# CompVis/stable-diffusion

Measured on AMD Instinct MI355X. Metric: 512x512 images/sec, SD-v1-4 50-step PLMS CFG=7.5, higher is better.
Workload: dtype f16

## Files before the change

stable-diffusion_amd/csrc/conv3halo.hip:

```cpp
#include "igemm_dev.h"

namespace sdmi {
namespace {

template <int BM, int BN, int WARPS_M, int WARPS_N, int NS>
__global__ void __launch_bounds__(WARPS_M* WARPS_N * 64) conv3halo_kernel(const IGemmParams p, const int tiles_m,
                                                                           const int tiles_n, const int chunks_per_split) {
#if defined(__HIP_DEVICE_COMPILE__)
  constexpr int NT = WARPS_M * WARPS_N * 64;
  constexpr int RPP = NT / 8;
  constexpr int PB = BN / RPP;
  constexpr int WTM = BM / WARPS_M, WTN = BN / WARPS_N;
  constexpr int TM = WTM / 32, TN = WTN / 32;
  constexpr int HPMAX = (BM / 64 + 2) * 66;
  constexpr int AHP = (HPMAX + RPP - 1) / RPP;
  constexpr int HALO_BYTES = AHP * RPP * 128;
  constexpr int BSTAGE = BN * 128;
  constexpr int LDS_BYTES = 2 * HALO_BYTES + NS * BSTAGE;
  constexpr int LASTA = 10 - NS;
  constexpr int PA = (AHP + LASTA) / (LASTA + 1);
  constexpr int KS = BK / 16;
  constexpr int G = (TM * TN >= 4) ? 1 : 2;
  constexpr int U = KS / G;
  constexpr int MPU = G * TM * TN;
  static_assert(PB >= 1 && TM >= 1 && TN >= 1 && RPP % 16 == 0 && NS >= 2 && NS <= 9, "tile/wave shape");
  static_assert(LDS_BYTES <= 160 * 1024, "LDS budget");

  __shared__ __attribute__((aligned(16))) unsigned char smem[LDS_BYTES];

  const int nblk = gridDim.x;
  const int bid = blockIdx.x;
  const int q8 = nblk >> 3, r8 = nblk & 7, xcd = bid & 7;
  const int wgid = (xcd < r8 ? xcd * (q8 + 1) : r8 * (q8 + 1) + (xcd - r8) * q8) + (bid >> 3);
  const int tiles_mn = tiles_m * tiles_n;
  const int split = wgid / tiles_mn;
  const int tmn = wgid - split * tiles_mn;
  int tile_m, tile_n;
  if (p.tile_n_fastest) { tile_m = tmn / tiles_n; tile_n = tmn - tile_m * tiles_n; }
  else { tile_n = tmn / tiles_m; tile_m = tmn - tile_n * tiles_m; }
  const int m0 = tile_m * BM, n0 = tile_n * BN;
  const int nch = (p.c0 + p.c1 + p.c2) / BK;
  const int c_begin = split * chunks_per_split;
  const int c_end = min(nch, c_begin + chunks_per_split);
  if (c_begin >= c_end) return;

  const int tid = threadIdx.x;
  SDMI_STAMP(dbg_t0);
  const int lane = tid & 63;
  const int wave = tid >> 6;
  const int cpos = tid & 7, lrow = tid >> 3;
  const int gch = cpos ^ ((lrow >> 1) & 7);
  const int wave_u = __builtin_amdgcn_readfirstlane(wave);
  const int wm = wave / WARPS_N, wn = wave - wm * WARPS_N;
  const int l31 = lane & 31, lg = lane >> 5;
  const int rsw = (l31 >> 1) & 7;

  const int W = p.Wout, H = p.Hout, HW = H * W, W2 = W + 2, ld = p.lda0;
  const int bimg = m0 / HW;
// ... 60 lines not shown
      for (int r = 0; r < 16; ++r) acc[i][j][r] = 0.f;

  auto a_base = [&](int i, int ky, int kx, int hbuf) -> int {
    const int rowt = hr0[i] + ky * W2 + kx;
    return hbuf * HALO_BYTES + ((rowt << 7) | ((lg ^ ((rowt >> 1) & 7)) << 4));
  };
  auto read_frags = [&](const int (&ab)[TM], int bstage, int ks, f16x8 (&a)[TM], f16x8 (&b)[TN]) {
#pragma unroll
    for (int i = 0; i < TM; ++i) a[i] = *(const f16x8*)(smem + (ab[i] ^ (ks << 5)));
    const unsigned char* st = smem + bstage * BSTAGE + b_lds + (((ks * 2 + lg) ^ rsw) << 4);
#pragma unroll
    for (int j = 0; j < TN; ++j) b[j] = *(const f16x8*)(st + j * 32 * 128);
  };
  auto mfma_step = [&](const f16x8 (&a)[TM], const f16x8 (&b)[TN]) {
#pragma unroll
    for (int i = 0; i < TM; ++i)
#pragma unroll
      for (int j = 0; j < TN; ++j) acc[i][j] = __builtin_amdgcn_mfma_f32_32x32x16_f16(a[i], b[j], acc[i][j], 0, 0, 0);
  };

  auto a_lo = [](int t) { return t <= LASTA ? (t * PA < AHP ? t * PA : AHP) : AHP; };
  auto a_hi = [](int t) { return t <= LASTA ? ((t + 1) * PA < AHP ? (t + 1) * PA : AHP) : AHP; };
  auto in_flight_ok = [&](int t) {
    int n = 0;
    for (int d = 0; d < NS - 2; ++d) { const int tt = (t - d + 18) % 9; n += a_hi(tt) - a_lo(tt) + PB; }
    return n;
  };

  const int kt_first = c_begin * 9, kt_last = c_end * 9 - 1;
  {
    const ChunkSrc cs = chunk_src(c_begin);
#pragma unroll
    for (int q = 0; q < AHP; ++q) issue_halo(cs, 0, q);
#pragma unroll
    for (int s2 = 0; s2 < NS - 1; ++s2) {
      const int vt = 9 - (NS - 1) + s2;
#pragma unroll
      for (int e = a_lo(vt); e < a_hi(vt); ++e) issue_halo(cs, 0, 0);
#pragma unroll
      for (int q = 0; q < PB; ++q) issue_b(min(kt_first + s2, kt_last), s2, q);
    }
  }
  wait_vmcnt_n(in_flight_ok(8));
  asm volatile("s_waitcnt lgkmcnt(0)\n\ts_barrier" ::: "memory");
  SDMI_STAMP(dbg_t1);
  f16x8 fa[2][G][TM], fb[2][G][TN];
  int ab[TM];
#pragma unroll
  for (int i = 0; i < TM; ++i) ab[i] = a_base(i, 0, 0, 0);
#pragma unroll
  for (int g = 0; g < G; ++g) read_frags(ab, 0, g, fa[0][g], fb[0][g]);

  int cur = 0, nxt = NS - 1, hb = 0;
  for (int c = c_begin; c < c_end; ++c) {
    const ChunkSrc csn = chunk_src(min(c + 1, c_end - 1));
#pragma unroll
    for (int tap = 0; tap < 9; ++tap) {
      const int kt = c * 9 + tap;
      const int tap1 = tap == 8 ? 0 : tap + 1;
      const int hb1 = tap == 8 ? (hb ^ 1) : hb;
      const int cur1 = (cur + 1 == NS) ? 0 : cur + 1;
      int ab1[TM];
#pragma unroll
      for (int i = 0; i < TM; ++i) ab1[i] = a_base(i, tap1 / 3, tap1 % 3, hb1);
      const int alo = a_lo(tap);
      const int na = a_hi(tap) - alo;
      const int npieces = na + PB;
      const int ppu = (npieces + U - 2) / (U - 1);
      const int bt = min(kt + NS - 1, kt_last);
#pragma unroll
      for (int u = 0; u < U; ++u) {
        if (u + 1 < U) {
#pragma unroll
          for (int g = 0; g < G; ++g) read_frags(ab, cur, (u + 1) * G + g, fa[(u + 1) & 1][g], fb[(u + 1) & 1][g]);
#pragma unroll
          for (int e = u * ppu; e < (u + 1) * ppu && e < npieces; ++e) {
            if (e < na) issue_halo(csn, hb ^ 1, alo + e);
            else issue_b(bt, nxt, e - na);
          }
        } else {
          wait_vmcnt_n(in_flight_ok(tap));
          asm volatile("s_waitcnt lgkmcnt(0)\n\ts_barrier" ::: "memory");
#pragma unroll
          for (int g = 0; g < G; ++g) read_frags(ab1, cur1, g, fa[0][g], fb[0][g]);
        }
#pragma unroll
        for (int g = 0; g < G; ++g) mfma_step(fa[u & 1][g], fb[u & 1][g]);
        __builtin_amdgcn_sched_group_barrier(0x100, G * (TM + TN), 0);
#pragma unroll
        for (int e = 0; e < MPU; ++e) {
          __builtin_amdgcn_sched_group_barrier(0x008, 1, 0);
          if (u + 1 < U && e < ppu && u * ppu + e < npieces) __builtin_amdgcn_sched_group_barrier(0x010, 1, 0);
        }
      }
#pragma unroll
      for (int i = 0; i < TM; ++i) ab[i] = ab1[i];
      cur = cur1;
      nxt = (nxt + 1 == NS) ? 0 : nxt + 1;
      hb = hb1;
    }
  }
  wait_vmcnt<0>();
  SDMI_STAMP(dbg_t2);
  igemm_epilogue<BM, BN, WARPS_M, WARPS_N, LDS_BYTES>(p, acc, m0, n0, split, tile_m, tile_n, smem);
#ifdef SDMI_IGEMM_TIMING
  if (p.dbg_times && tid == 0) {
    long long* d = p.dbg_times + 6 * (size_t)blockIdx.x;
    d[0] = dbg_t0; d[1] = dbg_t1; d[2] = dbg_t2; d[4] = (long long)__builtin_readcyclecounter();
  }
#endif
#endif
}

}

bool halo_supported(const IGemmParams& p, int bm) {
  const int W = p.Wout, HW = p.Hout * p.Wout;
  if (p.c0 % BK || p.c1 % BK || p.c2 % BK) return false;
  if (!(p.ksize == 3 && p.stride == 1 && p.pad == 1 && !p.up && p.Hin == p.Hout && p.Win == p.Wout && W >= 8 && W <= 64 &&
        (W & (W - 1)) == 0 && bm % W == 0))
    return false;
  const int cap = (((bm / 64 + 2) * 66 + bm / 4 - 1) / (bm / 4)) * (bm / 4);
  if (bm <= HW) return HW % bm == 0 && (bm / W + 2) * (W + 2) <= cap;
  return bm % HW == 0 && p.M % bm == 0 && (bm / HW) * (p.Hout + 2) * (W + 2) <= cap;
}

template <int BM, int BN, int WARPS_M, int WARPS_N, int NS>
int launch_halo_cfg(const IGemmParams& p, int splitk, hipStream_t stream) {
  SDMI_CHECK(halo_supported(p, BM), "halo-staged conv tile requested for an unsupported shape");
  const int tiles_m = cdiv(p.M, BM), tiles_n = cdiv(p.N, BN);
  const int nch = (p.c0 + p.c1 + p.c2) / BK;
  const int chunks_per_split = cdiv(nch, splitk);
  const int nsplit = cdiv(nch, chunks_per_split);
  IGemmParams q = p;
  q.splitk = nsplit;
  q.tile_n_fastest = tile_order_n_fastest(p);
  q.splitk_fused = 0;
  slab_layout(q, BM, BN, WARPS_M, WARPS_N, nsplit);
  q.epi_vec = epi_vec_ok(p);
  SDMI_CHECK(splitk_ws_need(p, BM, BN, nsplit) <= p.splitk_ws_floats, "split-K workspace too small");
  SDMI_CHECK((int64_t)p.M < (int64_t)65536 * p.Hout * p.Wout, "fast_div_hw: at most 65535 samples per launch");
  q.magic_hw = div_magic_hw(p.Hout * p.Wout);
  q.magic_w = div_magic(p.Wout);
  q.magic_w2 = div_magic(p.Wout + 2);
  q.log2w = 0;
  while ((1 << q.log2w) < p.Wout) ++q.log2w;
  {
    const int HW = p.Hout * p.Wout;
    q.halo_ipt = BM <= HW ? 1 : BM / HW;
    q.halo_thi = BM <= HW ? BM / p.Wout : p.Hout;
    q.magic_hpi = div_magic((q.halo_thi + 2) * (p.Wout + 2));
    const int tpi = q.halo_thi * p.Wout;
    q.log2_tpi = 0;
    while ((1 << q.log2_tpi) < tpi) ++q.log2_tpi;
    if (q.halo_ipt == 1) q.log2_tpi = 30;
  }
  for (int t = 0; t < p.gn_n; ++t) q.gn_magic[t] = div_magic(p.gn_cpg[t]);
  dim3 grid(tiles_m * tiles_n * nsplit), block(WARPS_M * WARPS_N * 64);
  static const int by_shape = env_int("SDMI_PROF_SHAPES", 0);
  std::string pname = std::string("conv3halo_") + std::to_string(BM) + "x" + std::to_string(BN) + "w" +
                      std::to_string(WARPS_M * WARPS_N) + "s" + std::to_string(NS);
  if (by_shape && prof_enabled())
    pname += "_M" + std::to_string(p.M) + "_N" + std::to_string(p.N) + "_K" + std::to_string(p.K) + "_s" + std::to_string(nsplit);
  const double src_pix = (double)p.B * p.Hin * p.Win;
  ProfScope ps(pname.c_str(), 2.0 * p.M * (double)p.N * p.K,
               src_pix * (p.c0 + p.c1) * 2.0 + (double)p.N * p.K * 2.0 + (double)p.M * p.N * ((p.out_f32 ? 4.0 : 0.0) + (p.out_f16 ? 2.0 : 0.0)) +
                   (p.residual ? (double)p.M * p.N * 4.0 : 0.0),
               stream);
  SDMI_LAUNCH((conv3halo_kernel<BM, BN, WARPS_M, WARPS_N, NS>), grid, block, 0, stream, q, tiles_m, tiles_n, chunks_per_split);
  SDMI_HIP_OK(hipGetLastError());
  ps.end();
  if (nsplit > 1) return launch_splitk_reduce(q, nsplit, stream);
  if (q.ln_out) return launch_layernorm(q.out_f32, q.ln_gamma, q.ln_beta, q.ln_out, q.M, q.N, q.ln_eps, stream);
  return 0;
}

int launch_halo_tile(int tile, const IGemmParams& p, int splitk, hipStream_t stream) {
  switch (tile) {
    case 14: return launch_halo_cfg<256, 64, 4, 2, 5>(p, splitk, stream);
    case 15: return launch_halo_cfg<256, 128, 4, 2, 3>(p, splitk, stream);
    case 16: return launch_halo_cfg<128, 64, 2, 2, 8>(p, splitk, stream);
    case 17: return launch_halo_cfg<128, 128, 2, 2, 5>(p, splitk, stream);
    default: return fail("not a halo-staged conv tile id");
  }
}

}
```

stable-diffusion_amd/csrc/gemm_split16.hip:

```cpp
#include "igemm_dev.h"

namespace sdmi {
namespace {

template <int BM, int BN, int WARPS_M, int WARPS_N, int NS, bool HALF>
__global__ void __launch_bounds__(WARPS_M* WARPS_N * 64) gemm_split16_kernel(const IGemmParams p, const int tiles_m, const int tiles_n,
                                                                               const int kt_per_split) {
#if defined(__HIP_DEVICE_COMPILE__)
  constexpr int NT = WARPS_M * WARPS_N * 64;
  constexpr int RPP = NT / 8;
  constexpr int A_PASSES = BM / RPP, B_PASSES = BN / RPP;
  constexpr int WTM = BM / WARPS_M, WTN = BN / WARPS_N;
  constexpr int TM = WTM / 32, TN = WTN / 32;
  constexpr int A_BYTES = BM * 128, B_BYTES = BN * 128;
  constexpr int STAGE_BYTES = 2 * (A_BYTES + B_BYTES);
  constexpr int LPT = 2 * (A_PASSES + B_PASSES);
  constexpr int KS = BK / 16;
  constexpr int PPU = (LPT + KS - 2) / (KS - 1);
  static_assert(A_PASSES >= 1 && B_PASSES >= 1 && TM >= 1 && TN >= 1 && RPP % 16 == 0 && NS >= 2, "tile/wave shape");
  static_assert(NS * STAGE_BYTES <= 160 * 1024, "LDS budget");

  __shared__ __attribute__((aligned(16))) unsigned char smem[NS * STAGE_BYTES];

  const int nblk = gridDim.x, bid = blockIdx.x;
  const int q8 = nblk >> 3, r8 = nblk & 7, xcd = bid & 7;
  const int wgid = (xcd < r8 ? xcd * (q8 + 1) : r8 * (q8 + 1) + (xcd - r8) * q8) + (bid >> 3);
  const int tiles_mn = tiles_m * tiles_n;
  const int split = wgid / tiles_mn;
  const int tmn = wgid - split * tiles_mn;
  int tile_m, tile_n;
  if (p.tile_n_fastest) { tile_m = tmn / tiles_n; tile_n = tmn - tile_m * tiles_n; }
  else { tile_n = tmn / tiles_m; tile_m = tmn - tile_n * tiles_m; }
  const int m0 = tile_m * BM, n0 = tile_n * BN;
  const int nkt = HALF ? p.nkt : p.K / BK;
  const int kt_begin = split * kt_per_split;
  const int kt_end = min(nkt, kt_begin + kt_per_split);
  if (kt_begin >= kt_end) return;

  const int tid = threadIdx.x;
  SDMI_STAMP(dbg_t0);
  const int lane = tid & 63, wave = tid >> 6;
  const int cpos = tid & 7, lrow = tid >> 3;
  const int gch = cpos ^ ((lrow >> 1) & 7);
  const int hi_oob = (HALF && gch >= 4) ? (int)0x80000000 : 0;
  const int kt_half = HALF ? nkt - 1 : -1;
  const int wave_u = __builtin_amdgcn_readfirstlane(wave);

  int a_off[A_PASSES], b_off[B_PASSES];
#pragma unroll
  for (int i = 0; i < A_PASSES; ++i) a_off[i] = (min(m0 + i * RPP + lrow, p.M - 1) * p.lda0 + gch * 8) * 2;
#pragma unroll
  for (int i = 0; i < B_PASSES; ++i) b_off[i] = (min(n0 + i * RPP + lrow, p.N - 1) * p.ldw + gch * 8) * 2;
  constexpr int OOB = (int)0x80000000;
  const __amdgpu_buffer_rsrc_t rsrc_hi = __builtin_amdgcn_make_buffer_rsrc((void*)p.a0, 0, OOB, 0x00020000);
  const __amdgpu_buffer_rsrc_t rsrc_lo = __builtin_amdgcn_make_buffer_rsrc((void*)p.a1, 0, OOB, 0x00020000);
  const __amdgpu_buffer_rsrc_t rsrc_w = __builtin_amdgcn_make_buffer_rsrc((void*)p.w, 0, OOB, 0x00020000);
  const int w_lo_off = 2 * p.K * 2;

  auto issue_piece = [&](int kt, int stage, int q) {
    const int soff = kt * (BK * 2);
    const int half = HALF ? (hi_oob & (kt == kt_half ? (int)0x80000000 : 0)) : 0;
    const bool isA = q < 2 * A_PASSES;
    const int qa = isA ? q : q - 2 * A_PASSES;
    const int npass = isA ? A_PASSES : B_PASSES;
    const int hl = qa >= npass ? 1 : 0, pass = qa - hl * npass;
    const unsigned row0 = (isA ? hl * BM : 2 * BM + hl * BN) + pass * RPP + wave_u * 8;
    auto dst = (__attribute__((address_space(3))) void*)(smem + stage * STAGE_BYTES + row0 * 128);
    if (isA) __builtin_amdgcn_raw_ptr_buffer_load_lds(hl ? rsrc_lo : rsrc_hi, dst, 16, a_off[pass] | half, soff, 0, 0);
    else __builtin_amdgcn_raw_ptr_buffer_load_lds(rsrc_w, dst, 16, b_off[pass] | half, soff + (hl ? w_lo_off : 0), 0, SDMI_W_AUX);
  };

  const int wm = wave / WARPS_N, wn = wave - wm * WARPS_N;
  const int l31 = lane & 31, lg = lane >> 5;
  const int rsw = (l31 >> 1) & 7;
  f32x16 acc[TM][TN];
#pragma unroll
  for (int i = 0; i < TM; ++i)
#pragma unroll
    for (int j = 0; j < TN; ++j)
#pragma unroll
      for (int r = 0; r < 16; ++r) acc[i][j][r] = 0.f;

  struct Frags { f16x8 ah[TM], al[TM], bh[TN], bl[TN]; };
  const int a_lds = (wm * WTM + l31) * 128, b_lds = 2 * A_BYTES + (wn * WTN + l31) * 128;
  auto read_frags = [&](int stage, int ks, Frags& f) {
    const unsigned char* st = smem + stage * STAGE_BYTES + (((ks * 2 + lg) ^ rsw) << 4);
#pragma unroll
    for (int i = 0; i < TM; ++i) {
      f.ah[i] = *(const f16x8*)(st + a_lds + i * 32 * 128);
      f.al[i] = *(const f16x8*)(st + a_lds + A_BYTES + i * 32 * 128);
    }
#pragma unroll
    for (int j = 0; j < TN; ++j) {
      f.bh[j] = *(const f16x8*)(st + b_lds + j * 32 * 128);
      f.bl[j] = *(const f16x8*)(st + b_lds + B_BYTES + j * 32 * 128);
    }
  };
  auto mfma_step = [&](const Frags& f) {
#pragma unroll
    for (int i = 0; i < TM; ++i)
#pragma unroll
      for (int j = 0; j < TN; ++j) {
        acc[i][j] = __builtin_amdgcn_mfma_f32_32x32x16_f16(f.ah[i], f.bh[j], acc[i][j], 0, 0, 0);
        acc[i][j] = __builtin_amdgcn_mfma_f32_32x32x16_f16(f.al[i], f.bh[j], acc[i][j], 0, 0, 0);
        acc[i][j] = __builtin_amdgcn_mfma_f32_32x32x16_f16(f.ah[i], f.bl[j], acc[i][j], 0, 0, 0);
      }
  };

  SDMI_STAMP(dbg_t1);
  int ld_kt = kt_begin;
  auto next_kt = [&]() { const int k = ld_kt; if (ld_kt + 1 < kt_end) ++ld_kt; return k; };
#pragma unroll
  for (int s = 0; s < NS - 1; ++s) {
    const int k = next_kt();
#pragma unroll
    for (int q = 0; q < LPT; ++q) issue_piece(k, s, q);
  }
  wait_vmcnt<LPT*(NS - 2)>();
  asm volatile("s_waitcnt lgkmcnt(0)\n\ts_barrier" ::: "memory");
  Frags fr[2];
  read_frags(0, 0, fr[0]);
  int cur = 0, nxt = NS - 1;
  for (int kt = kt_begin; kt < kt_end; ++kt) {
    const int kload = next_kt();
    const int cur1 = (cur + 1 == NS) ? 0 : cur + 1;
#pragma unroll
    for (int u = 0; u < KS; ++u) {
      if (u + 1 < KS) {
        read_frags(cur, u + 1, fr[(u + 1) & 1]);
#pragma unroll
        for (int q = u * PPU; q < (u + 1) * PPU && q < LPT; ++q) issue_piece(kload, nxt, q);
      } else {
        wait_vmcnt<LPT*(NS - 2)>();
        asm volatile("s_waitcnt lgkmcnt(0)\n\ts_barrier" ::: "memory");
        read_frags(cur1, 0, fr[0]);
      }
      mfma_step(fr[u & 1]);
      __builtin_amdgcn_sched_group_barrier(0x100, 2 * (TM + TN), 0);
#pragma unroll
      for (int e = 0; e < 3 * TM * TN; ++e) {
        __builtin_amdgcn_sched_group_barrier(0x008, 1, 0);
        if (u + 1 < KS && e < PPU && u * PPU + e < LPT) __builtin_amdgcn_sched_group_barrier(0x010, 1, 0);
      }
    }
    cur = cur1;
    nxt = (nxt + 1 == NS) ? 0 : nxt + 1;
  }
  wait_vmcnt<0>();
  SDMI_STAMP(dbg_t2);
  igemm_epilogue<BM, BN, WARPS_M, WARPS_N, NS * STAGE_BYTES>(p, acc, m0, n0, split, tile_m, tile_n, smem);
#ifdef SDMI_IGEMM_TIMING
  if (p.dbg_times && tid == 0) {
    long long* d = p.dbg_times + 6 * (size_t)blockIdx.x;
    d[0] = dbg_t0; d[1] = dbg_t1; d[2] = dbg_t2; d[4] = (long long)__builtin_readcyclecounter();
  }
#endif
#endif
}

template <int BM, int BN, int WARPS_M, int WARPS_N, int NS>
int launch_split16_cfg(const IGemmParams& p, int splitk, hipStream_t stream) {
  const int tiles_m = cdiv(p.M, BM), tiles_n = cdiv(p.N, BN);
  const int nkt = igemm_nkt(p);
  const int kt_per_split = cdiv(nkt, splitk);
  const int nsplit = cdiv(nkt, kt_per_split);
  IGemmParams q = p;
  q.nkt = nkt;
  q.splitk = nsplit;
  q.tile_n_fastest = tile_order_n_fastest(p);
  q.splitk_fused = 0;
  slab_layout(q, BM, BN, WARPS_M, WARPS_N, nsplit);
  q.epi_vec = epi_vec_ok(p);
  SDMI_CHECK(splitk_ws_need(p, BM, BN, nsplit) <= p.splitk_ws_floats, "split-K workspace too small");
  SDMI_CHECK((int64_t)p.M < (int64_t)65536 * p.Hout * p.Wout, "fast_div_hw: at most 65535 samples per launch");
  q.magic_hw = div_magic_hw(p.Hout * p.Wout);
  q.magic_w = div_magic(p.Wout);
  for (int t = 0; t < p.gn_n; ++t) q.gn_magic[t] = div_magic(p.gn_cpg[t]);
  dim3 grid(tiles_m * tiles_n * nsplit), block(WARPS_M * WARPS_N * 64);
  static const int by_shape = env_int("SDMI_PROF_SHAPES", 0);
  std::string pname = std::string("gemm_split16_") + std::to_string(BM) + "x" + std::to_string(BN) + "w" +
                      std::to_string(WARPS_M * WARPS_N) + "s" + std::to_string(NS);
  if (by_shape && prof_enabled())
    pname += "_M" + std::to_string(p.M) + "_N" + std::to_string(p.N) + "_K" + std::to_string(p.K) + "_s" + std::to_string(nsplit);
  ProfScope ps(pname.c_str(), 2.0 * p.M * (double)p.N * p.K,
               (double)p.M * p.K * 2.0 + (double)p.N * p.K * 2.0 + (double)p.M * p.N * ((p.out_f32 ? 4.0 : 0.0) + (p.out_f16 ? 2.0 : 0.0)) +
                   (p.residual ? (double)p.M * p.N * 4.0 : 0.0),
               stream, 6.0 * p.M * (double)p.N * p.K);
  if (igemm_has_half(p)) SDMI_LAUNCH((gemm_split16_kernel<BM, BN, WARPS_M, WARPS_N, NS, true>), grid, block, 0, stream, q, tiles_m, tiles_n, kt_per_split);
  else SDMI_LAUNCH((gemm_split16_kernel<BM, BN, WARPS_M, WARPS_N, NS, false>), grid, block, 0, stream, q, tiles_m, tiles_n, kt_per_split);
  SDMI_HIP_OK(hipGetLastError());
  ps.end();
  if (nsplit > 1) return launch_splitk_reduce(q, nsplit, stream);
  if (q.ln_out) return launch_layernorm(q.out_f32, q.ln_gamma, q.ln_beta, q.ln_out, q.M, q.N, q.ln_eps, stream);
  return 0;
}

}

bool split16_tile_supported(int tile) { return tile == 0 || tile == 1 || tile == 2 || tile == 4 || tile == 5 || tile == 8 || tile == 10; }

int launch_split16_tile(int tile, const IGemmParams& p, int splitk, hipStream_t stream) {
  SDMI_CHECK(p.a0 && p.a1 && p.ksize == 1 && p.mode == EPI_PLAIN && p.c1 == 0 && p.c2 == 0 && p.K == p.c0 && p.K % BKH == 0 &&
                 p.lda0 % 8 == 0 && p.ldw % 8 == 0 && p.ldw >= 3 * p.K,
             "split-fp16 GEMM: hi + lo operands, plain epilogue, K % 32 == 0, packed [N][3K] weights");
  switch (tile) {
    case 0: return launch_split16_cfg<128, 128, 2, 2, 2>(p, splitk, stream);
    case 1: return launch_split16_cfg<128, 64, 2, 2, 2>(p, splitk, stream);
    case 2: return launch_split16_cfg<64, 64, 2, 2, 2>(p, splitk, stream);
    case 4: return launch_split16_cfg<128, 64, 2, 2, 3>(p, splitk, stream);
    case 5: return launch_split16_cfg<64, 64, 2, 2, 3>(p, splitk, stream);
    case 8: return launch_split16_cfg<64, 128, 2, 2, 3>(p, splitk, stream);
    case 10: return launch_split16_cfg<64, 64, 2, 2, 4>(p, splitk, stream);
    default: return fail("split-fp16 GEMM: tile id without an instantiation");
  }
}

}
```

stable-diffusion_amd/csrc/igemm_dev.h:

```cpp
#pragma once
#include "common.h"
#include "prof.h"

namespace sdmi {
typedef unsigned u32x4 __attribute__((ext_vector_type(4)));

int launch_splitk_reduce(const IGemmParams& p, int nsplit, hipStream_t stream);
int launch_generic_tile_g0(int tile, const IGemmParams& p, bool dma, int splitk, hipStream_t stream);
int launch_generic_tile_g1(int tile, const IGemmParams& p, bool dma, int splitk, hipStream_t stream);
int launch_generic_tile_g2(int tile, const IGemmParams& p, bool dma, int splitk, hipStream_t stream);
int launch_generic_tile_h0(int tile, const IGemmParams& p, bool dma, int splitk, hipStream_t stream);
int launch_generic_tile_h1(int tile, const IGemmParams& p, bool dma, int splitk, hipStream_t stream);
int launch_generic_tile_h2(int tile, const IGemmParams& p, bool dma, int splitk, hipStream_t stream);

static int env_int(const char* name, int dflt) {
  const char* v = getenv(name);
  return v ? atoi(v) : dflt;
}

namespace {

constexpr int BK = 64;
constexpr int BKH = 32;
static inline int src_chunks(int c) { return (c + BK - 1) / BK; }
static inline bool igemm_has_half(const IGemmParams& p) { return p.split16 ? (p.K % BK != 0) : (p.c0 % BK || p.c1 % BK || p.c2 % BK); }
static inline int igemm_nkt(const IGemmParams& p) {
  if (p.split16) return src_chunks(p.K);
  return p.ksize * p.ksize * (src_chunks(p.c0) + src_chunks(p.c1) + src_chunks(p.c2));
}

#ifdef SDMI_IGEMM_TIMING
#define SDMI_STAMP(name) const long long name = p.dbg_times ? (long long)__builtin_readcyclecounter() : 0
#else
#define SDMI_STAMP(name)
#endif

__device__ __forceinline__ float gelu_erf(float x) {
  const float z = fabsf(x) * 0.70710678118654752440f;
  const float t = __builtin_amdgcn_rcpf(1.0f + 0.3275911f * z);
  const float poly = t * (0.254829592f + t * (-0.284496736f + t * (1.421413741f + t * (-1.453152027f + t * 1.061405429f))));
  const float erf_abs = 1.0f - poly * __expf(-z * z);
  const float erf_v = __builtin_copysignf(erf_abs, x);
  return 0.5f * x * (1.0f + erf_v);
}

__device__ __forceinline__ void wait_vmcnt_n(int n) {
  switch (n) {
#define SDMI_VMCNT_CASE(k) case k: asm volatile("s_waitcnt vmcnt(" #k ")" ::: "memory"); break
    SDMI_VMCNT_CASE(0); SDMI_VMCNT_CASE(1); SDMI_VMCNT_CASE(2); SDMI_VMCNT_CASE(3); SDMI_VMCNT_CASE(4);
    SDMI_VMCNT_CASE(5); SDMI_VMCNT_CASE(6); SDMI_VMCNT_CASE(7); SDMI_VMCNT_CASE(8); SDMI_VMCNT_CASE(9);
    SDMI_VMCNT_CASE(10); SDMI_VMCNT_CASE(11); SDMI_VMCNT_CASE(12); SDMI_VMCNT_CASE(13); SDMI_VMCNT_CASE(14);
    SDMI_VMCNT_CASE(15); SDMI_VMCNT_CASE(16); SDMI_VMCNT_CASE(17); SDMI_VMCNT_CASE(18); SDMI_VMCNT_CASE(19);
    SDMI_VMCNT_CASE(20); SDMI_VMCNT_CASE(21); SDMI_VMCNT_CASE(22); SDMI_VMCNT_CASE(23); SDMI_VMCNT_CASE(24);
    SDMI_VMCNT_CASE(25); SDMI_VMCNT_CASE(26); SDMI_VMCNT_CASE(27); SDMI_VMCNT_CASE(28); SDMI_VMCNT_CASE(29);
    SDMI_VMCNT_CASE(30); SDMI_VMCNT_CASE(31); SDMI_VMCNT_CASE(32); SDMI_VMCNT_CASE(33); SDMI_VMCNT_CASE(34);
    SDMI_VMCNT_CASE(35); SDMI_VMCNT_CASE(36); SDMI_VMCNT_CASE(37); SDMI_VMCNT_CASE(38); SDMI_VMCNT_CASE(39);
    SDMI_VMCNT_CASE(40); SDMI_VMCNT_CASE(41); SDMI_VMCNT_CASE(42); SDMI_VMCNT_CASE(43); SDMI_VMCNT_CASE(44);
    SDMI_VMCNT_CASE(45); SDMI_VMCNT_CASE(46); SDMI_VMCNT_CASE(47); SDMI_VMCNT_CASE(48);
#undef SDMI_VMCNT_CASE
    default: __builtin_trap();
  }
}
template <int N>
__device__ __forceinline__ void wait_vmcnt() {
  static_assert(N >= 0 && N <= 48, "add the literal");
  wait_vmcnt_n(N);
}

enum : int { KIND_1X1 = 0, KIND_3X3 = 1, KIND_3X3_UP = 2 };

__device__ __forceinline__ int fast_div(int m, unsigned long long magic) {
// ... 583 lines not shown
```

stable-diffusion_amd/csrc/igemm_kernel.h:

```cpp
#pragma once
#include <string>

#include "igemm_dev.h"

namespace sdmi {
namespace {


template <int BM, int BN, int WARPS_M, int WARPS_N, bool DMA, int NS, int KIND, bool HALF = false>
__global__ void __launch_bounds__(WARPS_M* WARPS_N * 64) igemm_kernel(const IGemmParams p, const int tiles_m,
                                                                       const int tiles_n, const int kt_per_split) {
  static_assert(DMA || NS == 2, "the register-staged path is double buffered");
#if defined(__HIP_DEVICE_COMPILE__)
  constexpr bool UP = KIND == KIND_3X3_UP;
  constexpr bool K3 = KIND != KIND_1X1;
  constexpr int NT = WARPS_M * WARPS_N * 64;
  constexpr int RPP = NT / 8;
  constexpr int A_PASSES = BM / RPP;
  constexpr int B_PASSES = BN / RPP;
  constexpr int WTM = BM / WARPS_M, WTN = BN / WARPS_N;
  constexpr int TM = WTM / 32, TN = WTN / 32;
  constexpr int STAGE_BYTES = (BM + BN) * 128;
  static_assert(A_PASSES >= 1 && B_PASSES >= 1 && TM >= 1 && TN >= 1, "tile/wave shape");
  static_assert(RPP % 16 == 0, "swizzle assumes pass offset keeps row bits 1..3");

  __shared__ __attribute__((aligned(16))) unsigned char smem[NS * STAGE_BYTES];

  const int nblk = gridDim.x;
  const int bid = blockIdx.x;
  const int q8 = nblk >> 3, r8 = nblk & 7, xcd = bid & 7;
  const int wgid = (xcd < r8 ? xcd * (q8 + 1) : r8 * (q8 + 1) + (xcd - r8) * q8) + (bid >> 3);
  const int tiles_mn = tiles_m * tiles_n;
  const int split = wgid / tiles_mn;
  const int tmn = wgid - split * tiles_mn;
  int tile_m, tile_n;
  if (p.tile_n_fastest) { tile_m = tmn / tiles_n; tile_n = tmn - tile_m * tiles_n; }
  else { tile_n = tmn / tiles_m; tile_m = tmn - tile_n * tiles_m; }
  const int m0 = tile_m * BM, n0 = tile_n * BN;
  const int nkt = HALF ? p.nkt : p.K / BK;
  const int kt_begin = split * kt_per_split;
  const int kt_end = min(nkt, kt_begin + kt_per_split);
  if (kt_begin >= kt_end) return;

  const int tid = threadIdx.x;
  SDMI_STAMP(dbg_t0);
  float2 lnf_pv[LNF_MAXP];
  float lnf_mean = 0.f, lnf_rstd = 1.f;
  const bool lnf_mine = p.lnf_part != nullptr && tid < BM;
  if (lnf_mine) lnf_request(p, min(m0 + tid, p.M - 1), lnf_pv);
  const int lane = tid & 63;
  const int wave = tid >> 6;
  const int cpos = tid & 7;
  const int lrow = tid >> 3;
  const int gch = cpos ^ ((lrow >> 1) & 7);
  const int hi_oob = (HALF && gch >= 4) ? (int)0x80000000 : 0;

  const int HWout = p.Hout * p.Wout;
  const int pad = K3 ? p.pad : 0;
  constexpr int ntap = K3 ? 9 : 1;
  const int ld = p.lda0;
  int a_off[A_PASSES];
  unsigned a_mask[K3 ? A_PASSES : 1];
// ... 51 lines not shown
  int ld_ky = K3 ? ld_tap / 3 : 0, ld_kx = K3 ? ld_tap - 3 * (ld_tap / 3) : 0;
  const int pc0 = p.c0, pc1 = p.c1, pc2 = p.c2;
  const int pp0 = (pc0 + BK - 1) & ~(BK - 1), pp01 = pp0 + ((pc1 + BK - 1) & ~(BK - 1));
  int ld_boff = 0;
  if constexpr (HALF) {
    const int dense0 = ld_cin0 - (ld_cin0 >= pp0 ? pp0 - pc0 : 0) - (ld_cin0 >= pp01 ? pp01 - pp0 - pc1 : 0);
    const int left = ld_cin0 < pp0 ? pc0 - ld_cin0 : (ld_cin0 < pp01 ? pc1 - (ld_cin0 - pp0) : pc2 - (ld_cin0 - pp01));
    ld_boff = (ntap * dense0 + ld_tap * min(left, BK)) * 2;
  }

  constexpr int OOB = (int)0x80000000;
  const long long a_shift = (K3 && !UP) ? (long long)(pad * p.Win + pad) * ld * 2 : 0;
  const char* const srcA0 = (const char*)p.a0 - a_shift; const char* const srcA1 = (const char*)p.a1 - a_shift;
  const char* const srcA2 = (const char*)p.a2 - a_shift;
  const __amdgpu_buffer_rsrc_t rsrc_w = __builtin_amdgcn_make_buffer_rsrc((void*)p.w, 0, OOB, 0x00020000);
  const int pWin = p.Win;

  struct TileCursor { __amdgpu_buffer_rsrc_t rsrc_a; int a_soff, b_soff; unsigned tapbit; int ky, kx; unsigned lds; int half; };
  auto next_tile = [&](int stage) {
    TileCursor c;
    const char* src; int coff, left;
    if (ld_cin0 < pp0) { src = srcA0; coff = ld_cin0; left = pc0 - coff; }
    else if (ld_cin0 < pp01) { src = srcA1; coff = ld_cin0 - pp0; left = pc1 - coff; }
    else { src = srcA2; coff = ld_cin0 - pp01; left = pc2 - coff; }
    const bool half = HALF && left < BK;
    c.rsrc_a = __builtin_amdgcn_make_buffer_rsrc((void*)src, 0, OOB, 0x00020000);
    c.a_soff = ((K3 && !UP) ? (ld_ky * pWin + ld_kx) * ld + coff : coff) * 2;
    c.b_soff = HALF ? ld_boff : ld_kt * (BK * 2);
    c.tapbit = 1u << (half ? ld_tap + 9 : ld_tap); c.ky = ld_ky; c.kx = ld_kx;
    c.half = half ? OOB : 0;
    c.lds = stage * STAGE_BYTES;
    if (ld_kt + 1 < kt_end) {
      ++ld_kt;
      if constexpr (HALF) ld_boff += half ? BKH * 2 : BK * 2;
      if constexpr (K3) {
        ++ld_tap;
        if (++ld_kx == 3) { ld_kx = 0; ++ld_ky; }
        if (ld_tap == ntap) { ld_tap = 0; ld_ky = 0; ld_kx = 0; ld_cin0 += BK; }
      } else {
        ld_cin0 += BK;
      }
    }
    return c;
  };
  auto a_voff = [&](const TileCursor& c, int i) -> int {
    int v;
    if constexpr (UP) v = a_ro[i][c.ky] + a_co[i][c.kx];
    else v = a_off[i];
    if constexpr (K3) v = (a_mask[i] & c.tapbit) ? v : OOB;
    else if constexpr (HALF) v |= hi_oob & c.half;
    return v;
  };
  auto b_voff = [&](const TileCursor& c, int i) -> int { return HALF ? (b_off[i] | (hi_oob & c.half)) : b_off[i]; };
  auto issue_piece = [&](const TileCursor& c, int q) {
    const unsigned row0 = (q < A_PASSES ? q * RPP : BM + (q - A_PASSES) * RPP) + wave_u * 8;
    auto dst = (__attribute__((address_space(3))) void*)(smem + c.lds + row0 * 128);
    if (q < A_PASSES) __builtin_amdgcn_raw_ptr_buffer_load_lds(c.rsrc_a, dst, 16, a_voff(c, q), c.a_soff, 0, 0);
    else __builtin_amdgcn_raw_ptr_buffer_load_lds(rsrc_w, dst, 16, b_voff(c, q - A_PASSES), c.b_soff, 0, SDMI_W_AUX);
  };
  auto issue_loads = [&](int stage) {
    const TileCursor c = next_tile(stage);
#pragma unroll
    for (int q = 0; q < A_PASSES + B_PASSES; ++q) {
      if constexpr (DMA) {
        issue_piece(c, q);
      } else {
        typedef int i32x4 __attribute__((ext_vector_type(4)));
        i32x4 v;
        if (q < A_PASSES) v = __builtin_amdgcn_raw_buffer_load_b128(c.rsrc_a, a_voff(c, q), c.a_soff, 0);
        else v = __builtin_amdgcn_raw_buffer_load_b128(rsrc_w, b_voff(c, q - A_PASSES), c.b_soff, 0);
        if (q < A_PASSES) regA[q] = __builtin_bit_cast(f16x8, v);
        else regB[q - A_PASSES] = __builtin_bit_cast(f16x8, v);
      }
    }
  };
  auto commit_regs = [&](int stage) {
    if constexpr (!DMA) {
      unsigned char* As = smem + stage * STAGE_BYTES;
      unsigned char* Bs = As + BM * 128;
#pragma unroll
      for (int i = 0; i < A_PASSES; ++i) *(f16x8*)(As + (i * RPP + lrow) * 128 + cpos * 16) = regA[i];
#pragma unroll
      for (int i = 0; i < B_PASSES; ++i) *(f16x8*)(Bs + (i * RPP + lrow) * 128 + cpos * 16) = regB[i];
    }
  };

  const int wm = wave / WARPS_N, wn = wave - wm * WARPS_N;
  const int l31 = lane & 31, lg = lane >> 5;
  const int rsw = (l31 >> 1) & 7;
  f32x16 acc[TM][TN];
#pragma unroll
  for (int i = 0; i < TM; ++i)
#pragma unroll
    for (int j = 0; j < TN; ++j)
#pragma unroll
      for (int r = 0; r < 16; ++r) acc[i][j][r] = 0.f;

  const int a_lds = (wm * WTM + l31) * 128, b_lds = BM * 128 + (wn * WTN + l31) * 128;
  auto read_frags = [&](int stage, int ks, f16x8 (&a)[TM], f16x8 (&b)[TN]) {
    const unsigned char* st = smem + stage * STAGE_BYTES + (((ks * 2 + lg) ^ rsw) << 4);
#pragma unroll
    for (int i = 0; i < TM; ++i) a[i] = *(const f16x8*)(st + a_lds + i * 32 * 128);
#pragma unroll
    for (int j = 0; j < TN; ++j) b[j] = *(const f16x8*)(st + b_lds + j * 32 * 128);
  };
  auto mfma_step = [&](const f16x8 (&a)[TM], const f16x8 (&b)[TN]) {
#pragma unroll
    for (int i = 0; i < TM; ++i)
#pragma unroll
      for (int j = 0; j < TN; ++j) acc[i][j] = __builtin_amdgcn_mfma_f32_32x32x16_f16(a[i], b[j], acc[i][j], 0, 0, 0);
  };

  SDMI_STAMP(dbg_t1);
  if constexpr (!DMA) { if (lnf_mine) lnf_finish(p, lnf_pv, &lnf_mean, &lnf_rstd); }
  if constexpr (DMA) {
    constexpr int LPT = A_PASSES + B_PASSES;
    constexpr int KS = BK / 16;
    constexpr int G = (TM * TN >= 4) ? 1 : 2;
    constexpr int U = KS / G;
    constexpr int PPU = (LPT + U - 2) / (U - 1);
    constexpr int MPU = G * TM * TN;
#pragma unroll
    for (int s = 0; s < NS - 1; ++s) issue_loads(s);
    if (p.lnf_part) { wait_vmcnt<0>(); if (lnf_mine) lnf_finish(p, lnf_pv, &lnf_mean, &lnf_rstd); }
    wait_vmcnt<LPT*(NS - 2)>();
    asm volatile("s_waitcnt lgkmcnt(0)\n\ts_barrier" ::: "memory");
    f16x8 fa[2][G][TM], fb[2][G][TN];
#pragma unroll
    for (int g = 0; g < G; ++g) read_frags(0, g, fa[0][g], fb[0][g]);
    int cur = 0, nxt = NS - 1;
    for (int kt = kt_begin; kt < kt_end; ++kt) {
      const TileCursor c = next_tile(nxt);
      const int cur1 = (cur + 1 == NS) ? 0 : cur + 1;
#pragma unroll
      for (int u = 0; u < U; ++u) {
        if (u + 1 < U) {
#pragma unroll
          for (int g = 0; g < G; ++g) read_frags(cur, (u + 1) * G + g, fa[(u + 1) & 1][g], fb[(u + 1) & 1][g]);
#pragma unroll
          for (int q = u * PPU; q < (u + 1) * PPU && q < LPT; ++q) issue_piece(c, q);
        } else {
          wait_vmcnt<LPT*(NS - 2)>();
          asm volatile("s_waitcnt lgkmcnt(0)\n\ts_barrier" ::: "memory");
#pragma unroll
          for (int g = 0; g < G; ++g) read_frags(cur1, g, fa[0][g], fb[0][g]);
        }
#pragma unroll
        for (int g = 0; g < G; ++g) mfma_step(fa[u & 1][g], fb[u & 1][g]);
        __builtin_amdgcn_sched_group_barrier(0x100, G * (TM + TN), 0);
#pragma unroll
        for (int e = 0; e < MPU; ++e) {
          __builtin_amdgcn_sched_group_barrier(0x008, 1, 0);
          if (u + 1 < U && e < PPU && u * PPU + e < LPT) __builtin_amdgcn_sched_group_barrier(0x010, 1, 0);
        }
      }
      cur = cur1;
      nxt = (nxt + 1 == NS) ? 0 : nxt + 1;
    }
    wait_vmcnt<0>();
  } else {
    issue_loads(0);
    commit_regs(0);
    for (int kt = kt_begin; kt < kt_end; ++kt) {
      const int cur = (kt - kt_begin) & 1;
      __syncthreads();
      const bool more = (kt + 1 < kt_end);
      if (more) issue_loads(cur ^ 1);
#pragma unroll
      for (int ks = 0; ks < BK / 16; ++ks) {
        f16x8 a[TM], b[TN];
        read_frags(cur, ks, a, b);
        mfma_step(a, b);
      }
      if (more) commit_regs(cur ^ 1);
    }
  }

  SDMI_STAMP(dbg_t2);
  igemm_epilogue<BM, BN, WARPS_M, WARPS_N, NS * STAGE_BYTES>(p, acc, m0, n0, split, tile_m, tile_n, smem, lnf_mean, lnf_rstd);
#ifdef SDMI_IGEMM_TIMING
  if (p.dbg_times && tid == 0) {
    long long* d = p.dbg_times + 6 * (size_t)blockIdx.x;
    d[0] = dbg_t0; d[1] = dbg_t1; d[2] = dbg_t2; d[4] = (long long)__builtin_readcyclecounter();
  }
#endif
#endif
}

template <int BM, int BN, int WARPS_M, int WARPS_N, int NS, bool HALF = false>
int launch_cfg(const IGemmParams& p, bool dma, int splitk, hipStream_t stream) {
  SDMI_CHECK(HALF || (p.c0 % BK == 0 && p.c1 % BK == 0 && p.c2 % BK == 0), "internal: a half k-tile launch on the whole-chunk kernel");
  const int tiles_m = cdiv(p.M, BM), tiles_n = cdiv(p.N, BN);
  const int nkt = igemm_nkt(p);
  const int kt_per_split = cdiv(nkt, splitk);
  const int nsplit = cdiv(nkt, kt_per_split);
  IGemmParams q = p;
  q.nkt = nkt;
  q.splitk = nsplit;
  q.tile_n_fastest = tile_order_n_fastest(p);
  q.splitk_fused = 0;
  slab_layout(q, BM, BN, WARPS_M, WARPS_N, nsplit);
  q.epi_vec = epi_vec_ok(p);
  SDMI_CHECK(splitk_ws_need(p, BM, BN, nsplit) <= p.splitk_ws_floats, "split-K workspace too small");
  SDMI_CHECK((int64_t)p.M < (int64_t)65536 * p.Hout * p.Wout, "fast_div_hw: at most 65535 samples per launch");
  q.magic_hw = div_magic_hw(p.Hout * p.Wout);
  q.magic_w = div_magic(p.Wout);
  for (int t = 0; t < p.gn_n; ++t) q.gn_magic[t] = div_magic(p.gn_cpg[t]);
  dim3 grid(tiles_m * tiles_n * nsplit), block(WARPS_M * WARPS_N * 64);
  static const int by_shape = env_int("SDMI_PROF_SHAPES", 0);
  std::string pname = std::string("igemm_") + std::to_string(BM) + "x" + std::to_string(BN) + "w" +
                      std::to_string(WARPS_M * WARPS_N) + "s" + std::to_string(NS) + (HALF ? "h" : "");
  if (by_shape && prof_enabled())
    pname += "_M" + std::to_string(p.M) + "_N" + std::to_string(p.N) + "_K" + std::to_string(p.K) + "_k" +
             std::to_string(p.ksize) + "_m" + std::to_string(p.mode) + "_s" + std::to_string(nsplit);
  const double src_pix = (double)p.B * p.Hin * p.Win;
  const double out_b = (p.out_f32 ? 4.0 : 0.0) + ((p.out_f16 || p.mode != EPI_PLAIN) ? 2.0 : 0.0);
  const double n_out = p.mode == EPI_GEGLU ? p.N / 2.0 : (double)p.N;
  const int k_alg = p.k_alg > 0 ? p.k_alg : p.K;
  const double cin_alg = p.k_alg > 0 ? (double)p.k_alg : (double)(p.c0 + p.c1 + p.c2);
  ProfScope ps(pname.c_str(), 2.0 * p.M * (double)p.N * k_alg,
               src_pix * cin_alg * 2.0 + (double)p.N * k_alg * 2.0 + (double)p.M * n_out * out_b +
                   (p.residual ? (double)p.M * p.N * 4.0 : 0.0),
               stream, 2.0 * p.M * (double)p.N * p.K);
  const int kind = p.ksize == 1 ? KIND_1X1 : (p.up ? KIND_3X3_UP : KIND_3X3);
#define SDMI_LAUNCH_KIND(K_)                                                                                        \
  do {                                                                                                              \
    if (dma) SDMI_LAUNCH((igemm_kernel<BM, BN, WARPS_M, WARPS_N, true, NS, K_, HALF>), grid, block, 0, stream, q,   \
                                tiles_m, tiles_n, kt_per_split);                                                    \
    else SDMI_LAUNCH((igemm_kernel<BM, BN, WARPS_M, WARPS_N, false, 2, K_, HALF>), grid, block, 0, stream, q,       \
                            tiles_m, tiles_n, kt_per_split);                                                        \
  } while (0)
  if (kind == KIND_1X1) SDMI_LAUNCH_KIND(KIND_1X1);
  else if (kind == KIND_3X3) SDMI_LAUNCH_KIND(KIND_3X3);
  else SDMI_LAUNCH_KIND(KIND_3X3_UP);
#undef SDMI_LAUNCH_KIND
  SDMI_HIP_OK(hipGetLastError());
  ps.end();
  if (nsplit > 1) return launch_splitk_reduce(q, nsplit, stream);
  if (q.ln_out) return launch_layernorm(q.out_f32, q.ln_gamma, q.ln_beta, q.ln_out, q.M, q.N, q.ln_eps, stream);
  return 0;
}

}
}
```

Measured before the change: 3.812.

## Peel pipeline tail to skip redundant clamped loads in GEMM/conv kernels

Adds a TAIL variant of the DMA-pipelined igemm, split16 GEMM and halo conv kernels. The main loop runs only while new k-tiles remain to fetch, and the last NS-1 tiles are drained without issuing the duplicate clamped loads the old loop kept issuing. Wait counts are adjusted per drain step and the final barrier-read is skipped. Short splits pad prologue loads out of bounds. The variant is on by default via an env var, at the cost of more template instantiations and intricate vmcnt bookkeeping that could be subtly wrong.

```diff
diff --git a/stable-diffusion_amd/csrc/conv3halo.hip b/stable-diffusion_amd/csrc/conv3halo.hip
--- a/stable-diffusion_amd/csrc/conv3halo.hip
+++ b/stable-diffusion_amd/csrc/conv3halo.hip
@@ -3,7 +3,7 @@
 namespace sdmi {
 namespace {
 
-template <int BM, int BN, int WARPS_M, int WARPS_N, int NS>
+template <int BM, int BN, int WARPS_M, int WARPS_N, int NS, bool TAIL>
 __global__ void __launch_bounds__(WARPS_M* WARPS_N * 64) conv3halo_kernel(const IGemmParams p, const int tiles_m,
                                                                            const int tiles_n, const int chunks_per_split) {
 #if defined(__HIP_DEVICE_COMPILE__)
@@ -170,6 +170,75 @@
   for (int g = 0; g < G; ++g) read_frags(ab, 0, g, fa[0][g], fb[0][g]);
 
   int cur = 0, nxt = NS - 1, hb = 0;
+  if constexpr (TAIL) {
+    auto in_flight_last = [&](int t) {
+      int n = 0;
+      for (int d = 0; d < NS - 2; ++d) {
+        const int tt = t - d;
+        if (tt >= 0) n += (tt + NS - 1 <= 8) ? PB : 0;
+        else n += a_hi(tt + 9) - a_lo(tt + 9) + PB;
+      }
+      return n;
+    };
+    auto tapstep = [&](const ChunkSrc& csn, const int c, const int tap, const bool lastc) __attribute__((always_inline)) {
+      const int kt = c * 9 + tap;
+      const int tap1 = tap == 8 ? 0 : tap + 1;
+      const int hb1 = tap == 8 ? (hb ^ 1) : hb;
+      const int cur1 = (cur + 1 == NS) ? 0 : cur + 1;
+      const bool last = lastc && tap == 8;
+      int ab1[TM];
+#pragma unroll
+      for (int i = 0; i < TM; ++i) ab1[i] = a_base(i, tap1 / 3, tap1 % 3, hb1);
+      const int alo = a_lo(tap);
+      const int na = lastc ? 0 : a_hi(tap) - alo;
+      const int nb = (lastc && tap + NS - 1 > 8) ? 0 : PB;
+      const int npieces = na + nb;
+      const int ppu = (npieces + U - 2) / (U - 1);
+      const int bt = kt + NS - 1;
+#pragma unroll
+      for (int u = 0; u < U; ++u) {
+        if (u + 1 < U) {
+#pragma unroll
+          for (int g = 0; g < G; ++g) read_frags(ab, cur, (u + 1) * G + g, fa[(u + 1) & 1][g], fb[(u + 1) & 1][g]);
+#pragma unroll
+          for (int e = u * ppu; e < (u + 1) * ppu && e < npieces; ++e) {
+            if (e < na) issue_halo(csn, hb ^ 1, alo + e);
+            else issue_b(bt, nxt, e - na);
+          }
+        } else {
+          if (!last) wait_vmcnt_n(lastc ? in_flight_last(tap) : in_flight_ok(tap));
+          asm volatile("s_waitcnt lgkmcnt(0)\n\ts_barrier" ::: "memory");
+          if (!last) {
+#pragma unroll
+            for (int g = 0; g < G; ++g) read_frags(ab1, cur1, g, fa[0][g], fb[0][g]);
+          }
+        }
+#pragma unroll
+        for (int g = 0; g < G; ++g) mfma_step(fa[u & 1][g], fb[u & 1][g]);
+        if (u + 1 < U || !last) __builtin_amdgcn_sched_group_barrier(0x100, G * (TM + TN), 0);
+#pragma unroll
+        for (int e = 0; e < MPU; ++e) {
+          __builtin_amdgcn_sched_group_barrier(0x008, 1, 0);
+          if (u + 1 < U && e < ppu && u * ppu + e < npieces) __builtin_amdgcn_sched_group_barrier(0x010, 1, 0);
+        }
+      }
+#pragma unroll
+      for (int i = 0; i < TM; ++i) ab[i] = ab1[i];
+      cur = cur1;
+      nxt = (nxt + 1 == NS) ? 0 : nxt + 1;
+      hb = hb1;
+    };
+    for (int c = c_begin; c < c_end - 1; ++c) {
+      const ChunkSrc csn = chunk_src(c + 1);
+#pragma unroll
+      for (int tap = 0; tap < 9; ++tap) tapstep(csn, c, tap, false);
+    }
+    {
+      const ChunkSrc csn = chunk_src(c_end - 1);
+#pragma unroll
+      for (int tap = 0; tap < 9; ++tap) tapstep(csn, c_end - 1, tap, true);
+    }
+  } else {
   for (int c = c_begin; c < c_end; ++c) {
     const ChunkSrc csn = chunk_src(min(c + 1, c_end - 1));
 #pragma unroll
@@ -219,6 +288,7 @@
     }
   }
   wait_vmcnt<0>();
+  }
   SDMI_STAMP(dbg_t2);
   igemm_epilogue<BM, BN, WARPS_M, WARPS_N, LDS_BYTES>(p, acc, m0, n0, split, tile_m, tile_n, smem);
 #ifdef SDMI_IGEMM_TIMING
@@ -285,7 +355,8 @@
                src_pix * (p.c0 + p.c1) * 2.0 + (double)p.N * p.K * 2.0 + (double)p.M * p.N * ((p.out_f32 ? 4.0 : 0.0) + (p.out_f16 ? 2.0 : 0.0)) +
                    (p.residual ? (double)p.M * p.N * 4.0 : 0.0),
                stream);
-  SDMI_LAUNCH((conv3halo_kernel<BM, BN, WARPS_M, WARPS_N, NS>), grid, block, 0, stream, q, tiles_m, tiles_n, chunks_per_split);
+  if (ring_tail_mode() != 0) SDMI_LAUNCH((conv3halo_kernel<BM, BN, WARPS_M, WARPS_N, NS, true>), grid, block, 0, stream, q, tiles_m, tiles_n, chunks_per_split);
+  else SDMI_LAUNCH((conv3halo_kernel<BM, BN, WARPS_M, WARPS_N, NS, false>), grid, block, 0, stream, q, tiles_m, tiles_n, chunks_per_split);
   SDMI_HIP_OK(hipGetLastError());
   ps.end();
   if (nsplit > 1) return launch_splitk_reduce(q, nsplit, stream);
diff --git a/stable-diffusion_amd/csrc/gemm_split16.hip b/stable-diffusion_amd/csrc/gemm_split16.hip
--- a/stable-diffusion_amd/csrc/gemm_split16.hip
+++ b/stable-diffusion_amd/csrc/gemm_split16.hip
@@ -3,7 +3,7 @@
 namespace sdmi {
 namespace {
 
-template <int BM, int BN, int WARPS_M, int WARPS_N, int NS, bool HALF>
+template <int BM, int BN, int WARPS_M, int WARPS_N, int NS, bool HALF, bool TAIL>
 __global__ void __launch_bounds__(WARPS_M* WARPS_N * 64) gemm_split16_kernel(const IGemmParams p, const int tiles_m, const int tiles_n,
                                                                                const int kt_per_split) {
 #if defined(__HIP_DEVICE_COMPILE__)
@@ -57,9 +57,9 @@
   const __amdgpu_buffer_rsrc_t rsrc_w = __builtin_amdgcn_make_buffer_rsrc((void*)p.w, 0, OOB, 0x00020000);
   const int w_lo_off = 2 * p.K * 2;
 
-  auto issue_piece = [&](int kt, int stage, int q) {
+  auto issue_piece = [&](int kt, int stage, int q, int pad = 0) {
     const int soff = kt * (BK * 2);
-    const int half = HALF ? (hi_oob & (kt == kt_half ? (int)0x80000000 : 0)) : 0;
+    const int half = (HALF ? (hi_oob & (kt == kt_half ? (int)0x80000000 : 0)) : 0) | pad;
     const bool isA = q < 2 * A_PASSES;
     const int qa = isA ? q : q - 2 * A_PASSES;
     const int npass = isA ? A_PASSES : B_PASSES;
@@ -110,6 +110,54 @@
   SDMI_STAMP(dbg_t1);
   int ld_kt = kt_begin;
   auto next_kt = [&]() { const int k = ld_kt; if (ld_kt + 1 < kt_end) ++ld_kt; return k; };
+  if constexpr (TAIL) {
+    const int ntile = kt_end - kt_begin;
+    const int npro = min(NS - 1, ntile);
+#pragma unroll
+    for (int s = 0; s < NS - 1; ++s) {
+      const int k = next_kt();
+      const int pad = s < ntile ? 0 : OOB;
+#pragma unroll
+      for (int q = 0; q < LPT; ++q) issue_piece(k, s, q, pad);
+    }
+    wait_vmcnt<LPT*(NS - 2)>();
+    asm volatile("s_waitcnt lgkmcnt(0)\n\ts_barrier" ::: "memory");
+    Frags fr[2];
+    read_frags(0, 0, fr[0]);
+    int cur = 0, nxt = NS - 1;
+    auto ktile = [&](const bool fetch, const int inflight, const bool last) __attribute__((always_inline)) {
+      const int kload = fetch ? next_kt() : 0;
+      const int cur1 = (cur + 1 == NS) ? 0 : cur + 1;
+#pragma unroll
+      for (int u = 0; u < KS; ++u) {
+        if (u + 1 < KS) {
+          read_frags(cur, u + 1, fr[(u + 1) & 1]);
+          if (fetch) {
+#pragma unroll
+            for (int q = u * PPU; q < (u + 1) * PPU && q < LPT; ++q) issue_piece(kload, nxt, q);
+          }
+        } else {
+          if (!last) wait_vmcnt_n(inflight);
+          asm volatile("s_waitcnt lgkmcnt(0)\n\ts_barrier" ::: "memory");
+          if (!last) read_frags(cur1, 0, fr[0]);
+        }
+        mfma_step(fr[u & 1]);
+        if (u + 1 < KS || !last) __builtin_amdgcn_sched_group_barrier(0x100, 2 * (TM + TN), 0);
+#pragma unroll
+        for (int e = 0; e < 3 * TM * TN; ++e) {
+          __builtin_amdgcn_sched_group_barrier(0x008, 1, 0);
+          if (fetch && u + 1 < KS && e < PPU && u * PPU + e < LPT) __builtin_amdgcn_sched_group_barrier(0x010, 1, 0);
+        }
+      }
+      cur = cur1;
+      nxt = (nxt + 1 == NS) ? 0 : nxt + 1;
+    };
+    for (int kt = kt_begin; kt < kt_end - (NS - 1); ++kt) ktile(true, LPT * (NS - 2), false);
+#pragma unroll
+    for (int j = 0; j < NS - 1; ++j)
+      if (j < npro) ktile(false, LPT * (NS - 3 - j > 0 ? NS - 3 - j : 0), j == NS - 2);
+    if (npro < NS - 1) wait_vmcnt<0>();
+  } else {
 #pragma unroll
   for (int s = 0; s < NS - 1; ++s) {
     const int k = next_kt();
@@ -147,6 +195,7 @@
     nxt = (nxt + 1 == NS) ? 0 : nxt + 1;
   }
   wait_vmcnt<0>();
+  }
   SDMI_STAMP(dbg_t2);
   igemm_epilogue<BM, BN, WARPS_M, WARPS_N, NS * STAGE_BYTES>(p, acc, m0, n0, split, tile_m, tile_n, smem);
 #ifdef SDMI_IGEMM_TIMING
@@ -186,8 +235,11 @@
                (double)p.M * p.K * 2.0 + (double)p.N * p.K * 2.0 + (double)p.M * p.N * ((p.out_f32 ? 4.0 : 0.0) + (p.out_f16 ? 2.0 : 0.0)) +
                    (p.residual ? (double)p.M * p.N * 4.0 : 0.0),
                stream, 6.0 * p.M * (double)p.N * p.K);
-  if (igemm_has_half(p)) SDMI_LAUNCH((gemm_split16_kernel<BM, BN, WARPS_M, WARPS_N, NS, true>), grid, block, 0, stream, q, tiles_m, tiles_n, kt_per_split);
-  else SDMI_LAUNCH((gemm_split16_kernel<BM, BN, WARPS_M, WARPS_N, NS, false>), grid, block, 0, stream, q, tiles_m, tiles_n, kt_per_split);
+  const bool half = igemm_has_half(p), ring_tail = ring_tail_mode() != 0;
+  if (half && ring_tail) SDMI_LAUNCH((gemm_split16_kernel<BM, BN, WARPS_M, WARPS_N, NS, true, true>), grid, block, 0, stream, q, tiles_m, tiles_n, kt_per_split);
+  else if (half) SDMI_LAUNCH((gemm_split16_kernel<BM, BN, WARPS_M, WARPS_N, NS, true, false>), grid, block, 0, stream, q, tiles_m, tiles_n, kt_per_split);
+  else if (ring_tail) SDMI_LAUNCH((gemm_split16_kernel<BM, BN, WARPS_M, WARPS_N, NS, false, true>), grid, block, 0, stream, q, tiles_m, tiles_n, kt_per_split);
+  else SDMI_LAUNCH((gemm_split16_kernel<BM, BN, WARPS_M, WARPS_N, NS, false, false>), grid, block, 0, stream, q, tiles_m, tiles_n, kt_per_split);
   SDMI_HIP_OK(hipGetLastError());
   ps.end();
   if (nsplit > 1) return launch_splitk_reduce(q, nsplit, stream);
diff --git a/stable-diffusion_amd/csrc/igemm_dev.h b/stable-diffusion_amd/csrc/igemm_dev.h
--- a/stable-diffusion_amd/csrc/igemm_dev.h
+++ b/stable-diffusion_amd/csrc/igemm_dev.h
@@ -17,6 +17,8 @@
   const char* v = getenv(name);
   return v ? atoi(v) : dflt;
 }
+
+static int ring_tail_mode() { return env_int("SDMI_RING_TAIL", 1); }
 
 namespace {
 
diff --git a/stable-diffusion_amd/csrc/igemm_kernel.h b/stable-diffusion_amd/csrc/igemm_kernel.h
--- a/stable-diffusion_amd/csrc/igemm_kernel.h
+++ b/stable-diffusion_amd/csrc/igemm_kernel.h
@@ -7,7 +7,7 @@
 namespace {
 
 
-template <int BM, int BN, int WARPS_M, int WARPS_N, bool DMA, int NS, int KIND, bool HALF = false>
+template <int BM, int BN, int WARPS_M, int WARPS_N, bool DMA, int NS, int KIND, bool HALF = false, bool TAIL = false>
 __global__ void __launch_bounds__(WARPS_M* WARPS_N * 64) igemm_kernel(const IGemmParams p, const int tiles_m,
                                                                        const int tiles_n, const int kt_per_split) {
   static_assert(DMA || NS == 2, "the register-staged path is double buffered");
@@ -165,11 +165,11 @@
     return v;
   };
   auto b_voff = [&](const TileCursor& c, int i) -> int { return HALF ? (b_off[i] | (hi_oob & c.half)) : b_off[i]; };
-  auto issue_piece = [&](const TileCursor& c, int q) {
+  auto issue_piece = [&](const TileCursor& c, int q, int pad = 0) {
     const unsigned row0 = (q < A_PASSES ? q * RPP : BM + (q - A_PASSES) * RPP) + wave_u * 8;
     auto dst = (__attribute__((address_space(3))) void*)(smem + c.lds + row0 * 128);
-    if (q < A_PASSES) __builtin_amdgcn_raw_ptr_buffer_load_lds(c.rsrc_a, dst, 16, a_voff(c, q), c.a_soff, 0, 0);
-    else __builtin_amdgcn_raw_ptr_buffer_load_lds(rsrc_w, dst, 16, b_voff(c, q - A_PASSES), c.b_soff, 0, SDMI_W_AUX);
+    if (q < A_PASSES) __builtin_amdgcn_raw_ptr_buffer_load_lds(c.rsrc_a, dst, 16, a_voff(c, q) | pad, c.a_soff, 0, 0);
+    else __builtin_amdgcn_raw_ptr_buffer_load_lds(rsrc_w, dst, 16, b_voff(c, q - A_PASSES) | pad, c.b_soff, 0, SDMI_W_AUX);
   };
   auto issue_loads = [&](int stage) {
     const TileCursor c = next_tile(stage);
@@ -233,6 +233,62 @@
     constexpr int U = KS / G;
     constexpr int PPU = (LPT + U - 2) / (U - 1);
     constexpr int MPU = G * TM * TN;
+    if constexpr (TAIL) {
+      const int ntile = kt_end - kt_begin;
+      const int npro = min(NS - 1, ntile);
+#pragma unroll
+      for (int s = 0; s < NS - 1; ++s) {
+        const TileCursor c = next_tile(s);
+        const int pad = s < ntile ? 0 : OOB;
+#pragma unroll
+        for (int q = 0; q < LPT; ++q) issue_piece(c, q, pad);
+      }
+      if (p.lnf_part) { wait_vmcnt<0>(); if (lnf_mine) lnf_finish(p, lnf_pv, &lnf_mean, &lnf_rstd); }
+      wait_vmcnt<LPT*(NS - 2)>();
+      asm volatile("s_waitcnt lgkmcnt(0)\n\ts_barrier" ::: "memory");
+      f16x8 fa[2][G][TM], fb[2][G][TN];
+#pragma unroll
+      for (int g = 0; g < G; ++g) read_frags(0, g, fa[0][g], fb[0][g]);
+      int cur = 0, nxt = NS - 1;
+      auto ktile = [&](const bool fetch, const int inflight, const bool last) __attribute__((always_inline)) {
+        TileCursor c;
+        if (fetch) c = next_tile(nxt);
+        const int cur1 = (cur + 1 == NS) ? 0 : cur + 1;
+#pragma unroll
+        for (int u = 0; u < U; ++u) {
+          if (u + 1 < U) {
+#pragma unroll
+            for (int g = 0; g < G; ++g) read_frags(cur, (u + 1) * G + g, fa[(u + 1) & 1][g], fb[(u + 1) & 1][g]);
+            if (fetch) {
+#pragma unroll
+              for (int q = u * PPU; q < (u + 1) * PPU && q < LPT; ++q) issue_piece(c, q);
+            }
+          } else {
+            if (!last) wait_vmcnt_n(inflight);
+            asm volatile("s_waitcnt lgkmcnt(0)\n\ts_barrier" ::: "memory");
+            if (!last) {
+#pragma unroll
+              for (int g = 0; g < G; ++g) read_frags(cur1, g, fa[0][g], fb[0][g]);
+            }
+          }
+#pragma unroll
+          for (int g = 0; g < G; ++g) mfma_step(fa[u & 1][g], fb[u & 1][g]);
+          if (u + 1 < U || !last) __builtin_amdgcn_sched_group_barrier(0x100, G * (TM + TN), 0);
+#pragma unroll
+          for (int e = 0; e < MPU; ++e) {
+            __builtin_amdgcn_sched_group_barrier(0x008, 1, 0);
+            if (fetch && u + 1 < U && e < PPU && u * PPU + e < LPT) __builtin_amdgcn_sched_group_barrier(0x010, 1, 0);
+          }
+        }
+        cur = cur1;
+        nxt = (nxt + 1 == NS) ? 0 : nxt + 1;
+      };
+      for (int kt = kt_begin; kt < kt_end - (NS - 1); ++kt) ktile(true, LPT * (NS - 2), false);
+#pragma unroll
+      for (int j = 0; j < NS - 1; ++j)
+        if (j < npro) ktile(false, LPT * (NS - 3 - j > 0 ? NS - 3 - j : 0), j == NS - 2);
+      if (npro < NS - 1) wait_vmcnt<0>();
+    } else {
 #pragma unroll
     for (int s = 0; s < NS - 1; ++s) issue_loads(s);
     if (p.lnf_part) { wait_vmcnt<0>(); if (lnf_mine) lnf_finish(p, lnf_pv, &lnf_mean, &lnf_rstd); }
@@ -271,6 +327,7 @@
       nxt = (nxt + 1 == NS) ? 0 : nxt + 1;
     }
     wait_vmcnt<0>();
+    }
   } else {
     issue_loads(0);
     commit_regs(0);
@@ -336,9 +393,12 @@
                    (p.residual ? (double)p.M * p.N * 4.0 : 0.0),
                stream, 2.0 * p.M * (double)p.N * p.K);
   const int kind = p.ksize == 1 ? KIND_1X1 : (p.up ? KIND_3X3_UP : KIND_3X3);
+  const bool ring_tail = ring_tail_mode() != 0;
 #define SDMI_LAUNCH_KIND(K_)                                                                                        \
   do {                                                                                                              \
-    if (dma) SDMI_LAUNCH((igemm_kernel<BM, BN, WARPS_M, WARPS_N, true, NS, K_, HALF>), grid, block, 0, stream, q,   \
+    if (dma && ring_tail) SDMI_LAUNCH((igemm_kernel<BM, BN, WARPS_M, WARPS_N, true, NS, K_, HALF, true>), grid, block, 0, \
+                                      stream, q, tiles_m, tiles_n, kt_per_split);                                   \
+    else if (dma) SDMI_LAUNCH((igemm_kernel<BM, BN, WARPS_M, WARPS_N, true, NS, K_, HALF>), grid, block, 0, stream, q, \
                                 tiles_m, tiles_n, kt_per_split);                                                    \
     else SDMI_LAUNCH((igemm_kernel<BM, BN, WARPS_M, WARPS_N, false, 2, K_, HALF>), grid, block, 0, stream, q,       \
                             tiles_m, tiles_n, kt_per_split);                                                        \
```

After: 3.826 (median of 6 runs). No clear change (+0.4%).
